# WoodsGao/pytorch_segmentation

Hardware: AMD Instinct MI355X
Metric: images/sec training step, DeepLabV3+ R50 512x512 21cl (higher is better)
Workload: dtype f32; 1 GPU; DeepLabV3+ ResNet-50 OS16, 21 classes, 512x512, batch 16 per GPU (BASELINE.json configs[2]); fwd + cross-entropy + bwd + SGD(momentum) step; global_batch=16, parallelism=dp1, conv_precision_policy=fp32, step_mode=eager

## Files before the change

### pytorch_segmentation_amd/csrc/norm_act.hip

```cpp
#include "common.h"
#include "half_io.h"

#include <stdlib.h>

namespace pseg {

constexpr int kMaxStatRows = 512;

static int stat_group(long long M, int C) {
  const int c4 = C / 4;
  const int tx = c4 >= 64 ? 64 : (c4 > 16 ? 32 : 16);
  const long long colblocks = (c4 + tx - 1) / tx;
  int r = kMaxStatRows;
  while (r > 32 && ((M + r - 1) / r) * colblocks < 1024) r >>= 1;
  return r;
}

template <typename T>
__device__ __forceinline__ f32x4 ld4(const T* p) { return ldv4(p); }
template <typename T>
__device__ __forceinline__ void st4(T* p, f32x4 v) { stv4(p, v); }

template <int V>
__device__ __forceinline__ fvec<V> act_mask_v(fvec<V> z, int act) {
// ... 74 lines not shown
}

template <int MODE, int NR, typename T, int V>
__global__ __launch_bounds__(256) void bn_bwd_reduce_kernel(const T* __restrict__ dz, int lddz,
                                                            const T* __restrict__ z, int ldz,
                                                            const T* __restrict__ y, int ldy,
                                                            const float* __restrict__ mean,
                                                            const float* __restrict__ invstd,
                                                            const float* __restrict__ scale,
                                                            const float* __restrict__ shift, int act, long long M, int C,
                                                            int R, float* __restrict__ pdb, float* __restrict__ pdg,
                                                            const uint32_t* __restrict__ mask) {
  PSEG_HELPER_PRIO();
  typedef fvec<V> vf;
  __shared__ vf sh[2][256];
  const int TX = blockDim.x, TY = blockDim.y;
  const int tx = threadIdx.x, ty = threadIdx.y;
  const int cv = blockIdx.y * TX + tx;
  const bool cok = cv * V < C;
  const long long r0 = (long long)blockIdx.x * R;
  const int nrows = (int)((r0 + R > M ? M : r0 + R) - r0);
  const int words = C >> 5;
  constexpr int ES = (int)sizeof(T);
  const __amdgpu_buffer_rsrc_t dzr = make_rsrc(dz + r0 * lddz, (uint32_t)(((long long)(nrows - 1) * lddz + C) * ES));
  const __amdgpu_buffer_rsrc_t yr = make_rsrc(y + r0 * ldy, (uint32_t)(((long long)(nrows - 1) * ldy + C) * ES));
  const __amdgpu_buffer_rsrc_t zr =
      make_rsrc(MODE == 2 ? z + r0 * ldz : y, MODE == 2 ? (uint32_t)(((long long)(nrows - 1) * ldz + C) * ES) : 0u);
  const __amdgpu_buffer_rsrc_t mr =
      make_rsrc(MODE == 1 ? mask + r0 * words : (const uint32_t*)y, MODE == 1 ? (uint32_t)(nrows * words * 4) : 0u);
  vf s = {}, q = {};
  if (cok) {
    const int c = cv * V;
    const vf mu = ldvec<V>(mean + c), is = ldvec<V>(invstd + c);
    vf sc = {}, sh4 = {};
    if (MODE == 3) {
      sc = ldvec<V>(scale + c);
      sh4 = ldvec<V>(shift + c);
    }
    const int vdz = (ty * lddz + c) * ES, vy = (ty * ldy + c) * ES, vz = (ty * ldz + c) * ES, vm = (ty * words + (c >> 5)) * 4;
    for (int base = 0; base < nrows; base += NR * TY) {
      vf g[NR], yv[NR];
#pragma unroll
      for (int k = 0; k < NR; ++k) {
        const int row = base + k * TY;
        g[k] = buf_ldvec<V, T>(dzr, vdz, row * lddz * ES);
        yv[k] = buf_ldvec<V, T>(yr, vy, row * ldy * ES);
      }
#pragma unroll
      for (int k = 0; k < NR; ++k) {
        const int row = base + k * TY;
        if (MODE == 1) {
          const uint32_t w = (uint32_t)__builtin_amdgcn_raw_buffer_load_b32(mr, vm, row * words * 4, 0);
          g[k] *= bits_to_mask<V>(w, c);
        } else if (MODE == 2) {
          g[k] *= act_mask_v<V>(buf_ldvec<V, T>(zr, vz, row * ldz * ES), act);
        } else if (MODE == 3) {
          g[k] *= act_mask_v<V>((yv[k] - mu) * sc + sh4, act);
        }
      }
      vf ts = g[0], tq = g[0] * ((yv[0] - mu) * is);
#pragma unroll
      for (int k = 1; k < NR; ++k) {
        ts += g[k];
        tq += g[k] * ((yv[k] - mu) * is);
      }
      s += ts;
      q += tq;
    }
  }
  sh[0][ty * TX + tx] = s;
  sh[1][ty * TX + tx] = q;
  __syncthreads();
  if (ty == 0 && cok) {
    vf ts = sh[0][tx], tq = sh[1][tx];
    for (int j = 1; j < TY; ++j) {
      ts += sh[0][j * TX + tx];
      tq += sh[1][j * TX + tx];
    }
    stvec<V>(pdb + (long long)blockIdx.x * C + cv * V, ts);
    stvec<V>(pdg + (long long)blockIdx.x * C + cv * V, tq);
  }
}

constexpr int kFinCh = 8, kFinLanes = 32, kFinLanesWide = 128;
constexpr int kFinWideRows = 128;

template <int LANES, int NQ>
__device__ __forceinline__ void lane_sum(double (*sh)[LANES][kFinCh], int ty, int lx, double (&v)[NQ]) {
#pragma unroll
  for (int q = 0; q < NQ; ++q) sh[q][ty][lx] = v[q];
  __syncthreads();
  constexpr int SEG = LANES >= 64 ? 16 : LANES;
  if (ty < LANES / SEG) {
#pragma unroll
    for (int q = 0; q < NQ; ++q) {
      double t = sh[q][ty * SEG][lx];
      for (int j = 1; j < SEG; ++j) t += sh[q][ty * SEG + j][lx];
      v[q] = t;
    }
  }
  if (LANES / SEG > 1) {
    __syncthreads();
    if (ty < LANES / SEG) {
#pragma unroll
      for (int q = 0; q < NQ; ++q) sh[q][ty][lx] = v[q];
    }
    __syncthreads();
    if (ty == 0) {
#pragma unroll
      for (int q = 0; q < NQ; ++q) {
        double t = sh[q][0][lx];
        for (int j = 1; j < LANES / SEG; ++j) t += sh[q][j][lx];
        v[q] = t;
      }
    }
  }
}

template <int LANES>
__device__ __forceinline__ void reduce_pair(const float* __restrict__ pa, const float* __restrict__ pb, int rows, int C,
                                            int c, int ty, double (*sh)[LANES][kFinCh], double& a, double& b) {
  const int lx = threadIdx.x % kFinCh;
  double v[2] = {0.0, 0.0};
  if (c < C) {
    int g = ty;
    for (; g + 3 * LANES < rows; g += 4 * LANES) {
      const float a0 = pa[(long long)g * C + c], a1 = pa[(long long)(g + LANES) * C + c],
                  a2 = pa[(long long)(g + 2 * LANES) * C + c], a3 = pa[(long long)(g + 3 * LANES) * C + c];
      float b0 = 0.f, b1 = 0.f, b2 = 0.f, b3 = 0.f;
      if (pb) {
        b0 = pb[(long long)g * C + c];
        b1 = pb[(long long)(g + LANES) * C + c];
        b2 = pb[(long long)(g + 2 * LANES) * C + c];
        b3 = pb[(long long)(g + 3 * LANES) * C + c];
      }
      v[0] += (double)a0;
      v[0] += (double)a1;
      v[0] += (double)a2;
      v[0] += (double)a3;
      if (pb) {
        v[1] += (double)b0;
        v[1] += (double)b1;
        v[1] += (double)b2;
        v[1] += (double)b3;
      }
    }
    for (; g < rows; g += LANES) {
      v[0] += (double)pa[(long long)g * C + c];
      if (pb) v[1] += (double)pb[(long long)g * C + c];
    }
  }
  lane_sum<LANES, 2>(sh, ty, lx, v);
  a = v[0];
  b = v[1];
}

__global__ __launch_bounds__(256) void stat_merge_kernel(const float* __restrict__ stat, int rows, int group,
                                                         long long count, int C, int per, float* __restrict__ out,
                                                         int out_rows) {
  PSEG_HELPER_PRIO();
  __shared__ double sh[2][kFinLanes][kFinCh];
  const int lx = threadIdx.x % kFinCh;
  const int c = blockIdx.x * kFinCh + lx;
  const int ty = threadIdx.x / kFinCh;
  const int g0 = blockIdx.y * per;
  int g1 = g0 + per;
  if (g1 > rows) g1 = rows;
  const long long plane = (long long)rows * C, oplane = (long long)out_rows * C;
  double s1 = 0.0, s2 = 0.0;
  float k0 = 0.f;
  if (c < C) {
    k0 = stat[(long long)g0 * C + c];
    for (int g = g0 + ty; g < g1; g += kFinLanes) {
      long long n = count - (long long)g * group;
      if (n > group) n = group;
      if (n <= 0) continue;
      const double d = (double)stat[(long long)g * C + c] - (double)k0;
      const double a = stat[plane + (long long)g * C + c], b = stat[2 * plane + (long long)g * C + c];
      s1 += a + (double)n * d;
      s2 += b + 2.0 * d * a + (double)n * d * d;
    }
  }
  sh[0][ty][lx] = s1;
  sh[1][ty][lx] = s2;
  __syncthreads();
  if (ty == 0 && c < C) {
    for (int j = 1; j < kFinLanes; ++j) {
      s1 += sh[0][j][lx];
      s2 += sh[1][j][lx];
    }
    const long long o = (long long)blockIdx.y * C + c;
    out[o] = k0;
    out[oplane + o] = (float)s1;
    out[2 * oplane + o] = (float)s2;
  }
}

template <int LANES>
__global__ __launch_bounds__(kFinCh * LANES) void bn_finalize_kernel(
    const float* __restrict__ stat, int rows, int group, long long count, int C, const float* __restrict__ gamma,
    const float* __restrict__ beta, float* __restrict__ rmean, float* __restrict__ rvar, float momentum, float eps,
    float* __restrict__ mean, float* __restrict__ invstd, float* __restrict__ scale, float* __restrict__ shift) {
  PSEG_HELPER_PRIO();
  __shared__ double sh[2][LANES][kFinCh];
  const int lx = threadIdx.x % kFinCh;
  const int c = blockIdx.x * kFinCh + lx;
  const int ty = threadIdx.x / kFinCh;
  const long long plane = (long long)rows * C;
  auto rows_of = [&](int g) -> long long {
    long long n = count - (long long)g * group;
    return n > group ? group : n;
  };
  double v[2] = {0.0, 0.0};
  double k0 = 0.0;
  if (c < C) {
    k0 = (double)stat[c];
    auto add = [&](int g, float kf, float s1f, float s2f) {
      const long long n = rows_of(g);
      if (n <= 0) return;
      const double d = (double)kf - k0, s1 = s1f;
      v[0] += s1 + (double)n * d;
      v[1] += (double)s2f + 2.0 * d * s1 + (double)n * d * d;
    };
    int g = ty;
    for (; g + 3 * LANES < rows; g += 4 * LANES) {
      float kk[4], ss1[4], ss2[4];
#pragma unroll
      for (int u = 0; u < 4; ++u) {
        const long long o = (long long)(g + u * LANES) * C + c;
        kk[u] = stat[o];
        ss1[u] = stat[plane + o];
        ss2[u] = stat[2 * plane + o];
      }
#pragma unroll
      for (int u = 0; u < 4; ++u) add(g + u * LANES, kk[u], ss1[u], ss2[u]);
    }
    for (; g < rows; g += LANES) {
      const long long o = (long long)g * C + c;
      add(g, stat[o], stat[plane + o], stat[2 * plane + o]);
    }
  }
  lane_sum<LANES, 2>(sh, ty, lx, v);
  if (ty == 0 && c < C) {
    const double n = (double)count;
    const double mu = k0 + v[0] / n;
    double M2 = v[1] - v[0] * v[0] / n;
    if (M2 < 0.0) M2 = 0.0;
    const double var = M2 / n;
    const float is = (float)(1.0 / sqrt(var + (double)eps));
    const float g = gamma ? gamma[c] : 1.f, b = beta ? beta[c] : 0.f;
    const float fm = (float)mu;
    mean[c] = fm;
    invstd[c] = is;
    const float sc = g * is;
    scale[c] = sc;
    shift[c] = b;
    if (rmean) rmean[c] = (1.f - momentum) * rmean[c] + momentum * fm;
    if (rvar) {
      const double unbiased = count > 1 ? M2 / (n - 1.0) : var;
      rvar[c] = (1.f - momentum) * rvar[c] + momentum * (float)unbiased;
    }
  }
}

template <int LANES>
__global__ __launch_bounds__(kFinCh * LANES) void bn_bwd_finalize_kernel(
    const float* __restrict__ pdb, const float* __restrict__ pdg, int rows, long long count, int C,
    float* __restrict__ dgamma, float* __restrict__ dbeta, int accumulate, int frozen, float* __restrict__ c1,
    float* __restrict__ c2) {
  PSEG_HELPER_PRIO();
  __shared__ double sh[2][LANES][kFinCh];
  const int c = blockIdx.x * kFinCh + (threadIdx.x % kFinCh);
  const int ty = threadIdx.x / kFinCh;
  double db, dg;
  reduce_pair<LANES>(pdb, pdg, rows, C, c, ty, sh, db, dg);
  if (ty == 0 && c < C) {
    const float fdb = (float)db, fdg = (float)dg;
    if (dbeta) dbeta[c] = accumulate ? dbeta[c] + fdb : fdb;
    if (dgamma) dgamma[c] = accumulate ? dgamma[c] + fdg : fdg;
    c1[c] = frozen ? 0.f : (float)(db / (double)count);
    c2[c] = frozen ? 0.f : (float)(dg / (double)count);
  }
}

template <int LANES>
__global__ __launch_bounds__(kFinCh * LANES) void col_reduce_kernel(const float* __restrict__ part, int rows, int C,
                                                                    float* __restrict__ out, int accumulate) {
  PSEG_HELPER_PRIO();
  __shared__ double sh[2][LANES][kFinCh];
  const int c = blockIdx.x * kFinCh + (threadIdx.x % kFinCh);
  const int ty = threadIdx.x / kFinCh;
  double s, unused;
  reduce_pair<LANES>(part, nullptr, rows, C, c, ty, sh, s, unused);
  if (ty == 0 && c < C) out[c] = accumulate ? out[c] + (float)s : (float)s;
}

__global__ void bn_eval_coeffs_kernel(const float* __restrict__ gamma, const float* __restrict__ beta,
                                      const float* __restrict__ rmean, const float* __restrict__ rvar, float eps, int C,
                                      float* __restrict__ mean, float* __restrict__ invstd, float* __restrict__ scale,
                                      float* __restrict__ shift) {
  PSEG_HELPER_PRIO();
  const int c = blockIdx.x * blockDim.x + threadIdx.x;
  if (c < C) {
    const float is = 1.f / sqrtf(rvar[c] + eps);
    mean[c] = rmean[c];
    invstd[c] = is;
    scale[c] = (gamma ? gamma[c] : 1.f) * is;
    shift[c] = beta ? beta[c] : 0.f;
  }
}

template <typename T, int V>
__global__ __launch_bounds__(256) void bn_act_fwd_kernel(const T* __restrict__ y, int ldy,
                                                         const float* __restrict__ mean, const float* __restrict__ scale,
                                                         const float* __restrict__ shift,
                                                         const T* __restrict__ res, int ldr, int act,
                                                         T* __restrict__ z, int ldz, uint32_t total, FastDiv cvdiv,
                                                         unsigned* __restrict__ amax, uint32_t* __restrict__ maskout) {
  PSEG_HELPER_PRIO();
  typedef fvec<V> vf;
  float vmax = 0.f;
  for (uint32_t i = blockIdx.x * 256u + threadIdx.x; i < total; i += gridDim.x * 256u) {
    const uint32_t r = cvdiv.div(i);
    const uint32_t c = (i - r * cvdiv.d) * V;
    vf v = ldvec<V>(y + (long long)r * ldy + c);
    if (scale) v = (v - ldvec<V>(mean + c)) * ldvec<V>(scale + c) + ldvec<V>(shift + c);
    if (res) v += ldvec<V>(res + (long long)r * ldr + c);
    if (maskout != nullptr) {
      vf vs = v;
      if constexpr (sizeof(T) == 2) vs = __builtin_convertvector(__builtin_convertvector(v, f16x8v), vf);
      const vf m = act_mask_v<V>(vs, act);
      uint32_t bits = 0;
#pragma unroll
      for (int k = 0; k < V; ++k) bits |= (m[k] != 0.f ? 1u : 0u) << k;
      bits <<= (c & 31);
#pragma unroll
      for (int o = 1; o < 32 / V; o <<= 1) bits |= __shfl_xor(bits, o, 64);
      if ((threadIdx.x & (32 / V - 1)) == 0) maskout[(long long)r * ((cvdiv.d * V) >> 5) + (c >> 5)] = bits;
    }
    if (act == PSEG_ACT_RELU) {
#pragma unroll
      for (int k = 0; k < V; ++k) v[k] = fmaxf(v[k], 0.f);
    } else if (act == PSEG_ACT_RELU6) {
#pragma unroll
      for (int k = 0; k < V; ++k) v[k] = fminf(fmaxf(v[k], 0.f), 6.f);
    }
    stvec<V>(z + (long long)r * ldz + c, v);
#pragma unroll
    for (int k = 0; k < V; ++k) vmax = fmaxf(vmax, fabsf(v[k]));
  }
  if (amax != nullptr) {
    __shared__ float shm[4];
#pragma unroll
    for (int o = 32; o > 0; o >>= 1) vmax = fmaxf(vmax, __shfl_xor(vmax, o, 64));
    if ((threadIdx.x & 63) == 0) shm[threadIdx.x >> 6] = vmax;
    __syncthreads();
    if (threadIdx.x == 0) {
      const float m = fmaxf(fmaxf(shm[0], shm[1]), fmaxf(shm[2], shm[3]));
      publish_amax(amax, m);
    }
  }
}

template <int NR, typename T, int V>
__global__ __launch_bounds__(256) void bn_act_fwd_rows_kernel(const T* __restrict__ y, int ldy,
                                                              const float* __restrict__ mean, const float* __restrict__ scale,
                                                              const float* __restrict__ shift, const T* __restrict__ res,
                                                              int ldr, int act, T* __restrict__ z, int ldz, long long M, int C,
                                                              int RB, uint32_t* __restrict__ maskout) {
  PSEG_HELPER_PRIO();
  typedef fvec<V> vf;
  const int TX = blockDim.x, TY = blockDim.y;
  const int tx = threadIdx.x, ty = threadIdx.y;
  const int cv = blockIdx.y * TX + tx;
  if (cv * V >= C) return;
  const int c = cv * V;
  const long long r0 = (long long)blockIdx.x * RB;
// ... 282 lines not shown
  {
    const int ch = threadIdx.x & (kSmallCh - 1), q = threadIdx.x / kSmallCh;
    const int c = c0 + ch;
    const bool cok = c < C;
    if (cok)
      for (int j = q; j < kFinLanes; j += 256 / kSmallCh) {
        double a = 0.0, b = 0.0;
        for (int g = j; g < rows; g += kFinLanes) {
          a += (double)pdb[(long long)g * C + c];
          b += (double)pdg[(long long)g * C + c];
        }
        s_pa[ch][j] = a;
        s_pb[ch][j] = b;
      }
    __syncthreads();
    if (q == 0) {
      float c1 = 0.f, c2 = 0.f;
      if (cok) {
        double db = 0.0, dg = 0.0;
        for (int j = 0; j < kFinLanes; ++j) {
          db += s_pa[ch][j];
          dg += s_pb[ch][j];
        }
        const float fdb = (float)db, fdg = (float)dg;
        if (blockIdx.x == 0) {
          if (dbeta) dbeta[c] = accumulate ? dbeta[c] + fdb : fdb;
          if (dgamma) dgamma[c] = accumulate ? dgamma[c] + fdg : fdg;
        }
        c1 = frozen ? 0.f : (float)(db / (double)count);
        c2 = frozen ? 0.f : (float)(dg / (double)count);
      }
      s_c1[ch] = c1;
      s_c2[ch] = c2;
    }
  }
  __syncthreads();
  const int tx = threadIdx.x & 15, ty = threadIdx.x >> 4;
  const int c = c0 + tx * 4;
  if (c >= C) return;
  const f32x4 c1 = ld4(&s_c1[tx * 4]), c2 = ld4(&s_c2[tx * 4]);
  const f32x4 mu = ld4(mean + c), is = ld4(invstd + c), sc = ld4(scale + c);
  f32x4 sh = {0.f, 0.f, 0.f, 0.f};
  if (shift) sh = ld4(shift + c);
  const long long r0 = (long long)blockIdx.x * kSmallRowsPerBlock;
  long long r1 = r0 + kSmallRowsPerBlock;
  if (r1 > M) r1 = M;
  for (long long r = r0 + ty; r < r1; r += 16) {
    f32x4 g = ld4(dz + r * lddz + c);
    const f32x4 yv = ld4(y + r * ldy + c);
    if (act != PSEG_ACT_NONE) g *= act_mask(z != nullptr ? ld4(z + r * ldz + c) : (yv - mu) * sc + sh, act);
    if (dres) {
      T* dp = dres + r * lddres + c;
      st4(dp, res_acc ? ld4(dp) + g : g);
    }
    const f32x4 xh = (yv - mu) * is;
    st4(dy + r * lddy + c, sc * (g - c1 - xh * c2));
  }
}

static bool al16(const void* p) { return ((uintptr_t)p & 15) == 0; }

static void stat_block(int C, dim3& block, dim3& grid, long long M, int R, int V = 4) {
  const int cv = C / V;
  const int tx = cv >= 64 ? 64 : (cv > 16 ? 32 : (cv > 8 ? 16 : 8));
  block = dim3(tx, 256 / tx);
  grid = dim3((unsigned)cdiv(M, R), (unsigned)cdiv(cv, tx));
}

template <typename T>
constexpr int lane_channels() { return sizeof(T) == 2 ? 8 : 4; }

static int ew_grid(long long total) {
  long long b = (total + 255) / 256;
  if (b > 256 * 8) b = 256 * 8;
  if (b < 1) b = 1;
  return (int)b;
}

#define EW_COMMON_CHECKS(name, M, C)                                                              \
  PSEG_REQUIRE((M) > 0 && (C) > 0 && (C) % 4 == 0, name ": need M > 0, C %% 4 == 0 (M=%lld C=%d)", \
               (long long)(M), (int)(C));                                                         \
  PSEG_REQUIRE((long long)(M) * ((C) / 4) < (1LL << 31), name ": tensor too large")

int launch_col_reduce(const float* part, int rows, int C, float* out, int accumulate, hipStream_t st) {
  if (rows >= kFinWideRows)
    hipLaunchKernelGGL(col_reduce_kernel<kFinLanesWide>, dim3(cdiv(C, kFinCh)), dim3(kFinCh * kFinLanesWide), 0, st, part,
                       rows, C, out, accumulate);
  else
    hipLaunchKernelGGL(col_reduce_kernel<kFinLanes>, dim3(cdiv(C, kFinCh)), dim3(kFinCh * kFinLanes), 0, st, part, rows, C,
                       out, accumulate);
  PSEG_LAUNCH_CHECK();
  return PSEG_OK;
}


template <typename T>
static bool ld_ok(int ld) { return ld % (sizeof(T) == 2 ? 8 : 4) == 0; }

template <typename T>
static int col_stats_impl(const T* y, int ldy, int64_t M, int C, float* stat, void* stream) {
  PSEG_REQUIRE(y && stat, "col_stats: null pointer");
  EW_COMMON_CHECKS("col_stats", M, C);
  PSEG_REQUIRE(ld_ok<T>(ldy) && al16(y) && al16(stat), "col_stats: alignment");
  dim3 block, grid;
  const int R = stat_group(M, C);
  stat_block(C, block, grid, M, R);
  hipLaunchKernelGGL((col_stats_kernel<true, T>), grid, block, 0, (hipStream_t)stream, y, ldy, (long long)M, C, R, stat,
                     (long long)cdiv(M, R) * C);
  PSEG_LAUNCH_CHECK();
  return PSEG_OK;
}

template <typename T>
static int bn_fwd_fused_impl(const float* stat, int rows, int group, int64_t count, int C, const float* gamma,
                             const float* beta, float* running_mean, float* running_var, float momentum, float eps,
                             float* mean, float* invstd, float* scale, float* shift, const T* y, int ldy, const T* residual,
                             int ldr, int act, T* z, int ldz, int64_t M, float* amax_z, void* stream) {
  PSEG_REQUIRE(stat && mean && invstd && scale && shift && y && z, "bn_fwd_fused: null pointer");
  PSEG_REQUIRE(rows > 0 && rows <= kSmallMaxPartials && group > 0 && count > 0, "bn_fwd_fused: bad sizes (rows %d)", rows);
  PSEG_REQUIRE((long long)rows * group >= count, "bn_fwd_fused: groups do not cover the rows");
  EW_COMMON_CHECKS("bn_fwd_fused", M, C);
  PSEG_REQUIRE(ld_ok<T>(ldy) && ld_ok<T>(ldz) && (!residual || ld_ok<T>(ldr)) && al16(y) && al16(z) && al16(residual),
               "bn_fwd_fused: alignment");
  const dim3 grid((unsigned)cdiv(M, kSmallRowsPerBlock), (unsigned)cdiv(C, kSmallCh));
  hipLaunchKernelGGL(bn_fwd_small_kernel<T>, grid, dim3(256), 0, (hipStream_t)stream, stat, rows, group, (long long)count,
                     C, gamma, beta, running_mean, running_var, momentum, eps, mean, invstd, scale, shift, y, ldy, residual,
                     ldr, act, z, ldz, (long long)M, (unsigned*)amax_z);
  PSEG_LAUNCH_CHECK();
  return PSEG_OK;
}

template <typename T>
static int bn_bwd_fused_impl(const float* part_db, const float* part_dg, int rows, int64_t count, int C, float* dgamma,
                             float* dbeta, int accumulate, int frozen, const T* dz, int lddz, const T* z, int ldz,
                             const T* y, int ldy, const float* mean, const float* invstd, const float* scale,
                             const float* shift, int act, T* dy, int lddy, T* dres, int lddres, int res_accumulate,
                             int64_t M, void* stream) {
  PSEG_REQUIRE(part_db && part_dg && dz && y && mean && invstd && scale && dy, "bn_bwd_fused: null pointer");
  PSEG_REQUIRE(rows > 0 && count > 0, "bn_bwd_fused: bad sizes");
  PSEG_REQUIRE(act == PSEG_ACT_NONE || z || shift, "bn_bwd_fused: activation needs z or shift");
  EW_COMMON_CHECKS("bn_bwd_fused", M, C);
  PSEG_REQUIRE(ld_ok<T>(lddz) && ld_ok<T>(ldy) && ld_ok<T>(lddy) && (!z || ld_ok<T>(ldz)) && (!dres || ld_ok<T>(lddres)) &&
                   al16(dz) && al16(z) && al16(y) && al16(dy) && al16(dres),
               "bn_bwd_fused: alignment");
  const dim3 grid((unsigned)cdiv(M, kSmallRowsPerBlock), (unsigned)cdiv(C, kSmallCh));
  hipLaunchKernelGGL(bn_bwd_small_kernel<T>, grid, dim3(256), 0, (hipStream_t)stream, part_db, part_dg, rows,
                     (long long)count, C, dgamma, dbeta, accumulate, frozen, dz, lddz, z, ldz, y, ldy, mean, invstd, scale,
                     shift, act, dy, lddy, dres, lddres, res_accumulate, (long long)M);
  PSEG_LAUNCH_CHECK();
  return PSEG_OK;
}

template <typename T>
static int bn_act_fwd_impl(const T* y, int ldy, const float* mean, const float* scale, const float* shift, const T* residual,
                           int ldr, int act, T* z, int ldz, int64_t M, int C, float* amax_z, uint32_t* mask_out,
                           void* stream) {
  PSEG_REQUIRE(y && z, "bn_act_fwd: null pointer");
  PSEG_REQUIRE(mask_out == nullptr || (C % 32 == 0 && act != PSEG_ACT_NONE), "bn_act_fwd: mask_out needs C %% 32 == 0 and an activation");
  PSEG_REQUIRE((scale == nullptr) == (shift == nullptr) && (scale == nullptr) == (mean == nullptr),
               "bn_act_fwd: mean/scale/shift must come together");
  EW_COMMON_CHECKS("bn_act_fwd", M, C);
  PSEG_REQUIRE(ld_ok<T>(ldy) && ld_ok<T>(ldz) && (!residual || ld_ok<T>(ldr)) && al16(y) && al16(z) && al16(residual) &&
                   al16(mean) && al16(scale) && al16(shift),
               "bn_act_fwd: alignment");
  constexpr int V = lane_channels<T>();
  const uint32_t total = (uint32_t)(M * (C / V));
  static const int rows_mode = [] {
    const char* e = getenv("PSEG_BN_FWD_ROWS");
    return e ? atoi(e) : 1;
  }();
  if constexpr (sizeof(T) == 2) {
    if (rows_mode != 0 && scale != nullptr && amax_z == nullptr && C % 8 == 0 && M >= 256 && (residual == nullptr || rows_mode == 2)) {
      dim3 block, grid;
// ... 95 lines not shown
                   al16(z) && al16(dy) && al16(dres) && al16(scale),
               "act_bwd: alignment");
  const uint32_t total = (uint32_t)(M * (C / 4));
  hipLaunchKernelGGL(act_bwd_kernel<T>, dim3(ew_grid(total)), dim3(256), 0, (hipStream_t)stream, dz, lddz, z, ldz, scale, act,
                     dy, lddy, dres, lddres, res_accumulate, total, FastDiv((uint32_t)(C / 4)));
  PSEG_LAUNCH_CHECK();
  return PSEG_OK;
}

template <typename T>
static int col_sum_impl(const T* dy, int ldy, int64_t M, int C, float* out, int accumulate, void* workspace,
                        int64_t workspace_bytes, void* stream) {
  PSEG_REQUIRE(dy && out, "col_sum: null pointer");
  EW_COMMON_CHECKS("col_sum", M, C);
  PSEG_REQUIRE(ld_ok<T>(ldy) && al16(dy) && al16(workspace), "col_sum: alignment");
  const int R = stat_group(M, C);
  const int rows = cdiv(M, R);
  const long long need = (long long)rows * C * 4;
  if (!workspace || workspace_bytes < need) {
    set_error("col_sum: needs %lld workspace bytes, got %lld", need, (long long)workspace_bytes);
    return PSEG_ERR_WORKSPACE;
  }
  dim3 block, grid;
  stat_block(C, block, grid, M, R);
  hipLaunchKernelGGL((col_stats_kernel<false, T>), grid, block, 0, (hipStream_t)stream, dy, ldy, (long long)M, C, R,
                     (float*)workspace, 0LL);
  PSEG_LAUNCH_CHECK();
  return launch_col_reduce((const float*)workspace, rows, C, out, accumulate, (hipStream_t)stream);
}

template <typename T>
static int copy2d_impl(const T* x, int ldx, T* y, int ldy, int64_t M, int C, int accumulate, void* stream) {
  PSEG_REQUIRE(x && y, "copy2d: null pointer");
  EW_COMMON_CHECKS("copy2d", M, C);
  PSEG_REQUIRE(ld_ok<T>(ldx) && ld_ok<T>(ldy) && al16(x) && al16(y), "copy2d: alignment");
  const uint32_t total = (uint32_t)(M * (C / 4));
  hipLaunchKernelGGL(copy2d_kernel<T>, dim3(ew_grid(total)), dim3(256), 0, (hipStream_t)stream, x, ldx, y, ldy, accumulate,
                     total, FastDiv((uint32_t)(C / 4)));
  PSEG_LAUNCH_CHECK();
  return PSEG_OK;
}

}

using namespace pseg;

#define HP(p) reinterpret_cast<const half_t*>(p)
#define HPM(p) reinterpret_cast<half_t*>(p)

extern "C" {

int pseg_col_stats_rows(int64_t M, int C) { return cdiv(M, stat_group(M, C)); }

int pseg_col_stats_group(int64_t M, int C) { return stat_group(M, C); }

int pseg_col_stats(const float* y, int ldy, int64_t M, int C, float* stat, void* stream) {
  return col_stats_impl<float>(y, ldy, M, C, stat, stream);
}
int pseg_col_stats_h(const pseg_half_t* y, int ldy, int64_t M, int C, float* stat, void* stream) {
  return col_stats_impl<half_t>(HP(y), ldy, M, C, stat, stream);
}

constexpr int kMergePer = 64;
constexpr int kTwoStageRows = 2048;

int64_t pseg_bn_finalize_workspace_bytes(int rows, int C) {
  return rows > kTwoStageRows ? (int64_t)3 * cdiv(rows, kMergePer) * C * 4 : 0;
}

int pseg_bn_finalize(const float* stat, int rows, int group, int64_t count, int C, const float* gamma,
                     const float* beta, float* running_mean, float* running_var, float momentum, float eps, float* mean,
                     float* invstd, float* scale, float* shift, void* workspace, int64_t workspace_bytes, void* stream) {
  PSEG_REQUIRE(stat && mean && invstd && scale && shift, "bn_finalize: null pointer");
  PSEG_REQUIRE(rows > 0 && group > 0 && count > 0 && C > 0, "bn_finalize: bad sizes");
  PSEG_REQUIRE((long long)rows * group >= count, "bn_finalize: %d groups of %d rows do not cover %lld rows", rows, group,
               (long long)count);
  if (rows > kTwoStageRows) {
    const int64_t need = pseg_bn_finalize_workspace_bytes(rows, C);
    if (!workspace || workspace_bytes < need) {
      set_error("bn_finalize: needs %lld workspace bytes, got %lld", (long long)need, (long long)workspace_bytes);
      return PSEG_ERR_WORKSPACE;
    }
    const int out_rows = cdiv(rows, kMergePer);
    hipLaunchKernelGGL(stat_merge_kernel, dim3(cdiv(C, kFinCh), out_rows), dim3(256), 0, (hipStream_t)stream, stat, rows,
                       group, (long long)count, C, kMergePer, (float*)workspace, out_rows);
    PSEG_LAUNCH_CHECK();
    stat = (const float*)workspace;
    rows = out_rows;
    group *= kMergePer;
  }
  if (rows >= kFinWideRows)
    hipLaunchKernelGGL(bn_finalize_kernel<kFinLanesWide>, dim3(cdiv(C, kFinCh)), dim3(kFinCh * kFinLanesWide), 0,
                       (hipStream_t)stream, stat, rows, group, (long long)count, C, gamma, beta, running_mean, running_var,
                       momentum, eps, mean, invstd, scale, shift);
  else
    hipLaunchKernelGGL(bn_finalize_kernel<kFinLanes>, dim3(cdiv(C, kFinCh)), dim3(kFinCh * kFinLanes), 0,
                       (hipStream_t)stream, stat, rows, group, (long long)count, C, gamma, beta, running_mean, running_var,
                       momentum, eps, mean, invstd, scale, shift);
  PSEG_LAUNCH_CHECK();
  return PSEG_OK;
}

int pseg_bn_small_path(int rows, int64_t M, int C) {
  static const int mode = [] {
    const char* e = getenv("PSEG_BN_SMALL");
    return e ? atoi(e) : 1;
  }();
  if (mode == 0) return 0;
  return (rows > 0 && rows <= kSmallMaxPartials && M * (int64_t)C <= (int64_t)(8 << 20)) ? 1 : 0;
}

int pseg_bn_fwd_fused(const float* stat, int rows, int group, int64_t count, int C, const float* gamma, const float* beta,
                      float* running_mean, float* running_var, float momentum, float eps, float* mean, float* invstd,
                      float* scale, float* shift, const float* y, int ldy, const float* residual, int ldr, int act,
                      float* z, int ldz, int64_t M, float* amax_z, void* stream) {
  return bn_fwd_fused_impl<float>(stat, rows, group, count, C, gamma, beta, running_mean, running_var, momentum, eps, mean,
                                  invstd, scale, shift, y, ldy, residual, ldr, act, z, ldz, M, amax_z, stream);
}
int pseg_bn_fwd_fused_h(const float* stat, int rows, int group, int64_t count, int C, const float* gamma, const float* beta,
                        float* running_mean, float* running_var, float momentum, float eps, float* mean, float* invstd,
                        float* scale, float* shift, const pseg_half_t* y, int ldy, const pseg_half_t* residual, int ldr,
                        int act, pseg_half_t* z, int ldz, int64_t M, void* stream) {
  return bn_fwd_fused_impl<half_t>(stat, rows, group, count, C, gamma, beta, running_mean, running_var, momentum, eps, mean,
                                   invstd, scale, shift, HP(y), ldy, HP(residual), ldr, act, HPM(z), ldz, M, nullptr, stream);
}

int pseg_bn_bwd_fused(const float* part_db, const float* part_dg, int rows, int64_t count, int C, float* dgamma,
                      float* dbeta, int accumulate, int frozen, const float* dz, int lddz, const float* z, int ldz,
                      const float* y, int ldy, const float* mean, const float* invstd, const float* scale,
                      const float* shift, int act, float* dy, int lddy, float* dres, int lddres, int res_accumulate,
                      int64_t M, void* stream) {
  return bn_bwd_fused_impl<float>(part_db, part_dg, rows, count, C, dgamma, dbeta, accumulate, frozen, dz, lddz, z, ldz, y,
                                  ldy, mean, invstd, scale, shift, act, dy, lddy, dres, lddres, res_accumulate, M, stream);
}
int pseg_bn_bwd_fused_h(const float* part_db, const float* part_dg, int rows, int64_t count, int C, float* dgamma,
                        float* dbeta, int accumulate, int frozen, const pseg_half_t* dz, int lddz, const pseg_half_t* z,
                        int ldz, const pseg_half_t* y, int ldy, const float* mean, const float* invstd, const float* scale,
                        const float* shift, int act, pseg_half_t* dy, int lddy, pseg_half_t* dres, int lddres,
                        int res_accumulate, int64_t M, void* stream) {
  return bn_bwd_fused_impl<half_t>(part_db, part_dg, rows, count, C, dgamma, dbeta, accumulate, frozen, HP(dz), lddz, HP(z),
                                   ldz, HP(y), ldy, mean, invstd, scale, shift, act, HPM(dy), lddy, HPM(dres), lddres,
                                   res_accumulate, M, stream);
}

int pseg_bn_eval_coeffs(const float* gamma, const float* beta, const float* running_mean, const float* running_var,
                        float eps, int C, float* mean, float* invstd, float* scale, float* shift, void* stream) {
  PSEG_REQUIRE(running_mean && running_var && mean && invstd && scale && shift && C > 0, "bn_eval_coeffs: bad argument");
  hipLaunchKernelGGL(bn_eval_coeffs_kernel, dim3(cdiv(C, 256)), dim3(256), 0, (hipStream_t)stream, gamma, beta,
                     running_mean, running_var, eps, C, mean, invstd, scale, shift);
  PSEG_LAUNCH_CHECK();
  return PSEG_OK;
}

int pseg_bn_act_fwd(const float* y, int ldy, const float* mean, const float* scale, const float* shift,
                    const float* residual, int ldr, int act, float* z, int ldz, int64_t M, int C, float* amax_z,
                    uint32_t* mask_out, void* stream) {
  return bn_act_fwd_impl<float>(y, ldy, mean, scale, shift, residual, ldr, act, z, ldz, M, C, amax_z, mask_out, stream);
}
int pseg_bn_act_fwd_h(const pseg_half_t* y, int ldy, const float* mean, const float* scale, const float* shift,
                      const pseg_half_t* residual, int ldr, int act, pseg_half_t* z, int ldz, int64_t M, int C,
                      uint32_t* mask_out, void* stream) {
  return bn_act_fwd_impl<half_t>(HP(y), ldy, mean, scale, shift, HP(residual), ldr, act, HPM(z), ldz, M, C, nullptr,
                                 mask_out, stream);
}

int pseg_bn_act_bwd_reduce(const float* dz, int lddz, const float* z, int ldz, const float* y, int ldy, const float* mean,
                           const float* invstd, const float* scale, const float* shift, int act, int64_t M, int C,
                           float* part_db, float* part_dg, const uint32_t* mask, void* stream) {
  return bn_act_bwd_reduce_impl<float>(dz, lddz, z, ldz, y, ldy, mean, invstd, scale, shift, act, M, C, part_db, part_dg,
                                       mask, stream);
}
int pseg_bn_act_bwd_reduce_h(const pseg_half_t* dz, int lddz, const pseg_half_t* z, int ldz, const pseg_half_t* y, int ldy,
                             const float* mean, const float* invstd, const float* scale, const float* shift, int act,
                             int64_t M, int C, float* part_db, float* part_dg, const uint32_t* mask, void* stream) {
  return bn_act_bwd_reduce_impl<half_t>(HP(dz), lddz, HP(z), ldz, HP(y), ldy, mean, invstd, scale, shift, act, M, C, part_db,
                                        part_dg, mask, stream);
}

int pseg_bn_bwd_finalize(const float* part_db, const float* part_dg, int rows, int64_t count, int C, float* dgamma,
                         float* dbeta, int accumulate, int frozen, float* c1, float* c2, void* stream) {
  PSEG_REQUIRE(part_db && part_dg && c1 && c2 && rows > 0 && count > 0 && C > 0, "bn_bwd_finalize: bad argument");
  if (rows >= kFinWideRows)
    hipLaunchKernelGGL(bn_bwd_finalize_kernel<kFinLanesWide>, dim3(cdiv(C, kFinCh)), dim3(kFinCh * kFinLanesWide), 0,
                       (hipStream_t)stream, part_db, part_dg, rows, (long long)count, C, dgamma, dbeta, accumulate, frozen, c1,
                       c2);
  else
    hipLaunchKernelGGL(bn_bwd_finalize_kernel<kFinLanes>, dim3(cdiv(C, kFinCh)), dim3(kFinCh * kFinLanes), 0,
                       (hipStream_t)stream, part_db, part_dg, rows, (long long)count, C, dgamma, dbeta, accumulate, frozen, c1,
                       c2);
  PSEG_LAUNCH_CHECK();
  return PSEG_OK;
}

int pseg_bn_act_bwd_apply(const float* dz, int lddz, const float* z, int ldz, const float* y, int ldy, const float* mean,
                          const float* invstd, const float* scale, const float* shift, const float* c1, const float* c2,
                          int act, float* dy, int lddy, float* dres, int lddres, int res_accumulate, int64_t M, int C,
                          const uint32_t* mask, uint16_t* dy_hi, uint16_t* dy_lo, int ldp, void* stream) {
  return bn_act_bwd_apply_impl<float>(dz, lddz, z, ldz, y, ldy, mean, invstd, scale, shift, c1, c2, act, dy, lddy, dres,
                                      lddres, res_accumulate, M, C, mask, dy_hi, dy_lo, ldp, stream);
}
int pseg_bn_act_bwd_apply_h(const pseg_half_t* dz, int lddz, const pseg_half_t* z, int ldz, const pseg_half_t* y, int ldy,
                            const float* mean, const float* invstd, const float* scale, const float* shift, const float* c1,
                            const float* c2, int act, pseg_half_t* dy, int lddy, pseg_half_t* dres, int lddres,
                            int res_accumulate, int64_t M, int C, const uint32_t* mask, void* stream) {
  return bn_act_bwd_apply_impl<half_t>(HP(dz), lddz, HP(z), ldz, HP(y), ldy, mean, invstd, scale, shift, c1, c2, act, HPM(dy),
                                       lddy, HPM(dres), lddres, res_accumulate, M, C, mask, nullptr, nullptr, 0, stream);
}

int pseg_act_bwd(const float* dz, int lddz, const float* z, int ldz, const float* scale, int act, float* dy, int lddy,
                 float* dres, int lddres, int res_accumulate, int64_t M, int C, void* stream) {
  return act_bwd_impl<float>(dz, lddz, z, ldz, scale, act, dy, lddy, dres, lddres, res_accumulate, M, C, stream);
}
int pseg_act_bwd_h(const pseg_half_t* dz, int lddz, const pseg_half_t* z, int ldz, const float* scale, int act,
                   pseg_half_t* dy, int lddy, pseg_half_t* dres, int lddres, int res_accumulate, int64_t M, int C,
                   void* stream) {
  return act_bwd_impl<half_t>(HP(dz), lddz, HP(z), ldz, scale, act, HPM(dy), lddy, HPM(dres), lddres, res_accumulate, M, C,
                              stream);
}

int pseg_col_sum(const float* dy, int ldy, int64_t M, int C, float* out, int accumulate, void* workspace,
                 int64_t workspace_bytes, void* stream) {
  return col_sum_impl<float>(dy, ldy, M, C, out, accumulate, workspace, workspace_bytes, stream);
}
int pseg_col_sum_h(const pseg_half_t* dy, int ldy, int64_t M, int C, float* out, int accumulate, void* workspace,
                   int64_t workspace_bytes, void* stream) {
  return col_sum_impl<half_t>(HP(dy), ldy, M, C, out, accumulate, workspace, workspace_bytes, stream);
}

int pseg_copy2d(const float* x, int ldx, float* y, int ldy, int64_t M, int C, int accumulate, void* stream) {
  return copy2d_impl<float>(x, ldx, y, ldy, M, C, accumulate, stream);
}
int pseg_copy2d_h(const pseg_half_t* x, int ldx, pseg_half_t* y, int ldy, int64_t M, int C, int accumulate, void* stream) {
  return copy2d_impl<half_t>(HP(x), ldx, HPM(y), ldy, M, C, accumulate, stream);
}

}
```

Baseline: 372.2 images/sec.

## Restructure BN finalize reductions with row-major lanes, float4 loads and wave shuffles

Reworks the batch-norm statistic merge, finalize, backward-finalize and column-reduce kernels so each lane walks rows for a group of channels. Loads become 16-byte vectors where C is divisible by 4 and pointers are aligned. Row counts are bucketed into compile-time unrolled variants so all loads issue before the double-precision accumulation. Cross-lane sums use wave shuffles instead of multi-stage shared-memory loops. The aim is to cut latency of these small launch-bound helper kernels that run for every BN layer, at the cost of many more template instantiations and more complex clamped-index and masking logic.

```diff
diff --git a/pytorch_segmentation_amd/csrc/norm_act.hip b/pytorch_segmentation_amd/csrc/norm_act.hip
--- a/pytorch_segmentation_amd/csrc/norm_act.hip
+++ b/pytorch_segmentation_amd/csrc/norm_act.hip
@@ -180,217 +180,303 @@
   }
 }
 
-constexpr int kFinCh = 8, kFinLanes = 32, kFinLanesWide = 128;
+constexpr int kFinThreads = 256, kFinLanes = 32, kFinLanesWide = 128;
 constexpr int kFinWideRows = 128;
 
-template <int LANES, int NQ>
-__device__ __forceinline__ void lane_sum(double (*sh)[LANES][kFinCh], int ty, int lx, double (&v)[NQ]) {
-#pragma unroll
-  for (int q = 0; q < NQ; ++q) sh[q][ty][lx] = v[q];
-  __syncthreads();
-  constexpr int SEG = LANES >= 64 ? 16 : LANES;
-  if (ty < LANES / SEG) {
-#pragma unroll
-    for (int q = 0; q < NQ; ++q) {
-      double t = sh[q][ty * SEG][lx];
-      for (int j = 1; j < SEG; ++j) t += sh[q][ty * SEG + j][lx];
-      v[q] = t;
-    }
-  }
-  if (LANES / SEG > 1) {
+template <int V>
+struct FinVec {
+  float x[V];
+};
+template <int V>
+__device__ __forceinline__ FinVec<V> fin_ld(const float* __restrict__ p) {
+  FinVec<V> r;
+  if constexpr (V == 4) {
+    const f32x4 t = *reinterpret_cast<const f32x4*>(p);
+    r.x[0] = t[0];
+    r.x[1] = t[1];
+    r.x[2] = t[2];
+    r.x[3] = t[3];
+  } else {
+    static_assert(V == 1, "one or four channels per lane");
+    r.x[0] = *p;
+  }
+  return r;
+}
+
+template <int LANES, int V>
+struct FinShape {
+  static constexpr int CG = kFinThreads / LANES;
+  static constexpr int CH = CG * V;
+  static constexpr int STRIDE = LANES + 1;
+  template <int NQ>
+  static constexpr int lds() { return LANES == kFinLanesWide ? (kFinThreads / 64) * NQ * V : NQ * V * CG * STRIDE; }
+};
+
+template <int LANES, int V, int NQ>
+__device__ __forceinline__ void lane_sum(double (&v)[NQ][V], double* __restrict__ sh, double (&out)[NQ]) {
+  typedef FinShape<LANES, V> S;
+  const int tid = threadIdx.x;
+  if constexpr (LANES == kFinLanesWide) {
+#pragma unroll
+    for (int o = 32; o > 0; o >>= 1) {
+#pragma unroll
+      for (int q = 0; q < NQ; ++q)
+#pragma unroll
+        for (int k = 0; k < V; ++k) v[q][k] += __shfl_xor(v[q][k], o, 64);
+    }
+    if ((tid & 63) == 0) {
+#pragma unroll
+      for (int q = 0; q < NQ; ++q)
+#pragma unroll
+        for (int k = 0; k < V; ++k) sh[(tid >> 6) * (NQ * V) + q * V + k] = v[q][k];
+    }
     __syncthreads();
-    if (ty < LANES / SEG) {
-#pragma unroll
-      for (int q = 0; q < NQ; ++q) sh[q][ty][lx] = v[q];
-    }
+    if (tid < S::CH) {
+      const int w = (tid / V) * (LANES / 64), k = tid % V;
+#pragma unroll
+      for (int q = 0; q < NQ; ++q) out[q] = sh[w * (NQ * V) + q * V + k] + sh[(w + 1) * (NQ * V) + q * V + k];
+    }
+  } else {
+    static_assert(NQ * S::CH <= 64, "one wave adds the lane sums");
+    const int ty = tid % LANES, cg = tid / LANES;
+#pragma unroll
+    for (int q = 0; q < NQ; ++q)
+#pragma unroll
+      for (int k = 0; k < V; ++k) sh[((q * V + k) * S::CG + cg) * S::STRIDE + ty] = v[q][k];
     __syncthreads();
-    if (ty == 0) {
-#pragma unroll
-      for (int q = 0; q < NQ; ++q) {
-        double t = sh[q][0][lx];
-        for (int j = 1; j < LANES / SEG; ++j) t += sh[q][j][lx];
-        v[q] = t;
-      }
-    }
-  }
-}
-
-template <int LANES>
-__device__ __forceinline__ void reduce_pair(const float* __restrict__ pa, const float* __restrict__ pb, int rows, int C,
-                                            int c, int ty, double (*sh)[LANES][kFinCh], double& a, double& b) {
-  const int lx = threadIdx.x % kFinCh;
-  double v[2] = {0.0, 0.0};
-  if (c < C) {
-    int g = ty;
-    for (; g + 3 * LANES < rows; g += 4 * LANES) {
-      const float a0 = pa[(long long)g * C + c], a1 = pa[(long long)(g + LANES) * C + c],
-                  a2 = pa[(long long)(g + 2 * LANES) * C + c], a3 = pa[(long long)(g + 3 * LANES) * C + c];
-      float b0 = 0.f, b1 = 0.f, b2 = 0.f, b3 = 0.f;
-      if (pb) {
-        b0 = pb[(long long)g * C + c];
-        b1 = pb[(long long)(g + LANES) * C + c];
-        b2 = pb[(long long)(g + 2 * LANES) * C + c];
-        b3 = pb[(long long)(g + 3 * LANES) * C + c];
-      }
-      v[0] += (double)a0;
-      v[0] += (double)a1;
-      v[0] += (double)a2;
-      v[0] += (double)a3;
-      if (pb) {
-        v[1] += (double)b0;
-        v[1] += (double)b1;
-        v[1] += (double)b2;
-        v[1] += (double)b3;
-      }
-    }
-    for (; g < rows; g += LANES) {
-      v[0] += (double)pa[(long long)g * C + c];
-      if (pb) v[1] += (double)pb[(long long)g * C + c];
-    }
-  }
-  lane_sum<LANES, 2>(sh, ty, lx, v);
-  a = v[0];
-  b = v[1];
-}
-
-__global__ __launch_bounds__(256) void stat_merge_kernel(const float* __restrict__ stat, int rows, int group,
-                                                         long long count, int C, int per, float* __restrict__ out,
-                                                         int out_rows) {
+    if (tid < 64) {
+      double t = 0.0;
+      if (tid < NQ * S::CH) {
+        const int ch = tid % S::CH, q = tid / S::CH;
+        const double* p = sh + ((q * V + ch % V) * S::CG + ch / V) * S::STRIDE;
+        t = p[0];
+#pragma unroll 8
+        for (int j = 1; j < LANES; ++j) t += p[j];
+      }
+#pragma unroll
+      for (int q = 0; q < NQ; ++q) out[q] = __shfl(t, (tid % S::CH) + q * S::CH, 64);
+    }
+  }
+}
+
+static int fin_bucket(int rows, int lanes) {
+  for (int nr = 2; nr <= 16; nr *= 2)
+    if (rows <= nr * lanes) return nr;
+  return 0;
+}
+
+template <int LANES, int V, int NR, int NQ>
+__device__ __forceinline__ void reduce_rows(const float* __restrict__ pa, const float* __restrict__ pb, int rows, int C,
+                                            int cv, int ty, double (&v)[NQ][V]) {
+  constexpr int B = NR > 0 ? NR : 4;
+  for (int base = 0; base < (NR > 0 ? 1 : rows); base += B * LANES) {
+    FinVec<V> a[B], b[NQ == 2 ? B : 1];
+#pragma unroll
+    for (int u = 0; u < B; ++u) {
+      const int g = base + ty + u * LANES;
+      const long long o = (long long)(g < rows ? g : rows - 1) * C + cv;
+      a[u] = fin_ld<V>(pa + o);
+      if constexpr (NQ == 2) b[u] = fin_ld<V>(pb + o);
+    }
+    __builtin_amdgcn_sched_barrier(0);
+#pragma unroll
+    for (int u = 0; u < B; ++u) {
+      const bool ok = base + ty + u * LANES < rows;
+#pragma unroll
+      for (int k = 0; k < V; ++k) {
+        v[0][k] += (double)(ok ? a[u].x[k] : 0.f);
+        if constexpr (NQ == 2) v[1][k] += (double)(ok ? b[u].x[k] : 0.f);
+      }
+    }
+  }
+}
+
+template <int V>
+__global__ __launch_bounds__(kFinThreads) void stat_merge_kernel(const float* __restrict__ stat, int rows, int group,
+                                                                 long long count, int C, float* __restrict__ out,
+                                                                 int out_rows) {
   PSEG_HELPER_PRIO();
-  __shared__ double sh[2][kFinLanes][kFinCh];
-  const int lx = threadIdx.x % kFinCh;
-  const int c = blockIdx.x * kFinCh + lx;
-  const int ty = threadIdx.x / kFinCh;
+  constexpr int NR = 2, per = NR * kFinLanes;
+  const int ty = threadIdx.x % kFinLanes;
+  const int cv = (blockIdx.x * (kFinThreads / kFinLanes) + threadIdx.x / kFinLanes) * V;
   const int g0 = blockIdx.y * per;
-  int g1 = g0 + per;
-  if (g1 > rows) g1 = rows;
+  const int g1 = g0 + per < rows ? g0 + per : rows;
   const long long plane = (long long)rows * C, oplane = (long long)out_rows * C;
-  double s1 = 0.0, s2 = 0.0;
-  float k0 = 0.f;
-  if (c < C) {
-    k0 = stat[(long long)g0 * C + c];
-    for (int g = g0 + ty; g < g1; g += kFinLanes) {
+  double s1[V], s2[V];
+#pragma unroll
+  for (int k = 0; k < V; ++k) s1[k] = s2[k] = 0.0;
+  FinVec<V> k0 = {};
+  if (cv < C) {
+    FinVec<V> kk[NR], a[NR], b[NR];
+    k0 = fin_ld<V>(stat + (long long)g0 * C + cv);
+#pragma unroll
+    for (int u = 0; u < NR; ++u) {
+      const int g = g0 + ty + u * kFinLanes;
+      const long long o = (long long)(g < g1 ? g : g1 - 1) * C + cv;
+      kk[u] = fin_ld<V>(stat + o);
+      a[u] = fin_ld<V>(stat + plane + o);
+      b[u] = fin_ld<V>(stat + 2 * plane + o);
+    }
+    __builtin_amdgcn_sched_barrier(0);
+#pragma unroll
+    for (int u = 0; u < NR; ++u) {
+      const int g = g0 + ty + u * kFinLanes;
       long long n = count - (long long)g * group;
       if (n > group) n = group;
-      if (n <= 0) continue;
-      const double d = (double)stat[(long long)g * C + c] - (double)k0;
-      const double a = stat[plane + (long long)g * C + c], b = stat[2 * plane + (long long)g * C + c];
-      s1 += a + (double)n * d;
-      s2 += b + 2.0 * d * a + (double)n * d * d;
-    }
-  }
-  sh[0][ty][lx] = s1;
-  sh[1][ty][lx] = s2;
-  __syncthreads();
-  if (ty == 0 && c < C) {
-    for (int j = 1; j < kFinLanes; ++j) {
-      s1 += sh[0][j][lx];
-      s2 += sh[1][j][lx];
-    }
-    const long long o = (long long)blockIdx.y * C + c;
-    out[o] = k0;
-    out[oplane + o] = (float)s1;
-    out[2 * oplane + o] = (float)s2;
-  }
-}
-
-template <int LANES>
-__global__ __launch_bounds__(kFinCh * LANES) void bn_finalize_kernel(
+      const bool ok = g < g1 && n > 0;
+      if (!ok) n = 0;
+#pragma unroll
+      for (int k = 0; k < V; ++k) {
+        const double d = (double)(ok ? kk[u].x[k] : k0.x[k]) - (double)k0.x[k], sa = ok ? a[u].x[k] : 0.f;
+        s1[k] += sa + (double)n * d;
+        s2[k] += (double)(ok ? b[u].x[k] : 0.f) + 2.0 * d * sa + (double)n * d * d;
+      }
+    }
+  }
+#pragma unroll
+  for (int o = kFinLanes / 2; o > 0; o >>= 1) {
+#pragma unroll
+    for (int k = 0; k < V; ++k) {
+      s1[k] += __shfl_xor(s1[k], o, 64);
+      s2[k] += __shfl_xor(s2[k], o, 64);
+    }
+  }
+  if (ty == 0 && cv < C) {
+    const long long o = (long long)blockIdx.y * C + cv;
+#pragma unroll
+    for (int k = 0; k < V; ++k) {
+      out[o + k] = k0.x[k];
+      out[oplane + o + k] = (float)s1[k];
+      out[2 * oplane + o + k] = (float)s2[k];
+    }
+  }
+}
+
+template <int LANES, int V, int NR>
+__global__ __launch_bounds__(kFinThreads) void bn_finalize_kernel(
     const float* __restrict__ stat, int rows, int group, long long count, int C, const float* __restrict__ gamma,
     const float* __restrict__ beta, float* __restrict__ rmean, float* __restrict__ rvar, float momentum, float eps,
     float* __restrict__ mean, float* __restrict__ invstd, float* __restrict__ scale, float* __restrict__ shift) {
   PSEG_HELPER_PRIO();
-  __shared__ double sh[2][LANES][kFinCh];
-  const int lx = threadIdx.x % kFinCh;
-  const int c = blockIdx.x * kFinCh + lx;
-  const int ty = threadIdx.x / kFinCh;
+  typedef FinShape<LANES, V> S;
+  __shared__ double sh[S::template lds<2>()];
+  const int ty = threadIdx.x % LANES;
+  const int cv = blockIdx.x * S::CH + (threadIdx.x / LANES) * V;
+  const int c = blockIdx.x * S::CH + threadIdx.x;
+  const bool fin = threadIdx.x < S::CH && c < C;
   const long long plane = (long long)rows * C;
-  auto rows_of = [&](int g) -> long long {
-    long long n = count - (long long)g * group;
-    return n > group ? group : n;
-  };
-  double v[2] = {0.0, 0.0};
-  double k0 = 0.0;
-  if (c < C) {
-    k0 = (double)stat[c];
-    auto add = [&](int g, float kf, float s1f, float s2f) {
-      const long long n = rows_of(g);
-      if (n <= 0) return;
-      const double d = (double)kf - k0, s1 = s1f;
-      v[0] += s1 + (double)n * d;
-      v[1] += (double)s2f + 2.0 * d * s1 + (double)n * d * d;
-    };
-    int g = ty;
-    for (; g + 3 * LANES < rows; g += 4 * LANES) {
-      float kk[4], ss1[4], ss2[4];
-#pragma unroll
-      for (int u = 0; u < 4; ++u) {
-        const long long o = (long long)(g + u * LANES) * C + c;
-        kk[u] = stat[o];
-        ss1[u] = stat[plane + o];
-        ss2[u] = stat[2 * plane + o];
-      }
-#pragma unroll
-      for (int u = 0; u < 4; ++u) add(g + u * LANES, kk[u], ss1[u], ss2[u]);
-    }
-    for (; g < rows; g += LANES) {
-      const long long o = (long long)g * C + c;
-      add(g, stat[o], stat[plane + o], stat[2 * plane + o]);
-    }
-  }
-  lane_sum<LANES, 2>(sh, ty, lx, v);
-  if (ty == 0 && c < C) {
+  float ek0 = 0.f, eg = 1.f, eb = 0.f, erm = 0.f, erv = 0.f;
+  if (fin) {
+    ek0 = stat[c];
+    if (gamma) eg = gamma[c];
+    if (beta) eb = beta[c];
+    if (rmean) erm = rmean[c];
+    if (rvar) erv = rvar[c];
+  }
+  double v[2][V];
+#pragma unroll
+  for (int k = 0; k < V; ++k) v[0][k] = v[1][k] = 0.0;
+  if (cv < C) {
+    constexpr int B = NR > 0 ? NR : 4;
+    const FinVec<V> k0 = fin_ld<V>(stat + cv);
+    for (int base = 0; base < (NR > 0 ? 1 : rows); base += B * LANES) {
+      FinVec<V> kk[B], a[B], b[B];
+#pragma unroll
+      for (int u = 0; u < B; ++u) {
+        const int g = base + ty + u * LANES;
+        const long long o = (long long)(g < rows ? g : rows - 1) * C + cv;
+        kk[u] = fin_ld<V>(stat + o);
+        a[u] = fin_ld<V>(stat + plane + o);
+        b[u] = fin_ld<V>(stat + 2 * plane + o);
+      }
+      __builtin_amdgcn_sched_barrier(0);
+#pragma unroll
+      for (int u = 0; u < B; ++u) {
+        const int g = base + ty + u * LANES;
+        long long n = count - (long long)g * group;
+        if (n > group) n = group;
+        const bool ok = g < rows && n > 0;
+        if (!ok) n = 0;
+#pragma unroll
+        for (int k = 0; k < V; ++k) {
+          const double d = (double)(ok ? kk[u].x[k] : k0.x[k]) - (double)k0.x[k], s1 = ok ? a[u].x[k] : 0.f;
+          v[0][k] += s1 + (double)n * d;
+          v[1][k] += (double)(ok ? b[u].x[k] : 0.f) + 2.0 * d * s1 + (double)n * d * d;
+        }
+      }
+    }
+  }
+  double s[2];
+  lane_sum<LANES, V, 2>(v, sh, s);
+  if (fin) {
     const double n = (double)count;
-    const double mu = k0 + v[0] / n;
-    double M2 = v[1] - v[0] * v[0] / n;
+    const double mu = (double)ek0 + s[0] / n;
+    double M2 = s[1] - s[0] * s[0] / n;
     if (M2 < 0.0) M2 = 0.0;
     const double var = M2 / n;
     const float is = (float)(1.0 / sqrt(var + (double)eps));
-    const float g = gamma ? gamma[c] : 1.f, b = beta ? beta[c] : 0.f;
     const float fm = (float)mu;
     mean[c] = fm;
     invstd[c] = is;
-    const float sc = g * is;
-    scale[c] = sc;
-    shift[c] = b;
-    if (rmean) rmean[c] = (1.f - momentum) * rmean[c] + momentum * fm;
+    scale[c] = eg * is;
+    shift[c] = eb;
+    if (rmean) rmean[c] = (1.f - momentum) * erm + momentum * fm;
     if (rvar) {
       const double unbiased = count > 1 ? M2 / (n - 1.0) : var;
-      rvar[c] = (1.f - momentum) * rvar[c] + momentum * (float)unbiased;
-    }
-  }
-}
-
-template <int LANES>
-__global__ __launch_bounds__(kFinCh * LANES) void bn_bwd_finalize_kernel(
+      rvar[c] = (1.f - momentum) * erv + momentum * (float)unbiased;
+    }
+  }
+}
+
+template <int LANES, int V, int NR>
+__global__ __launch_bounds__(kFinThreads) void bn_bwd_finalize_kernel(
     const float* __restrict__ pdb, const float* __restrict__ pdg, int rows, long long count, int C,
     float* __restrict__ dgamma, float* __restrict__ dbeta, int accumulate, int frozen, float* __restrict__ c1,
     float* __restrict__ c2) {
   PSEG_HELPER_PRIO();
-  __shared__ double sh[2][LANES][kFinCh];
-  const int c = blockIdx.x * kFinCh + (threadIdx.x % kFinCh);
-  const int ty = threadIdx.x / kFinCh;
-  double db, dg;
-  reduce_pair<LANES>(pdb, pdg, rows, C, c, ty, sh, db, dg);
-  if (ty == 0 && c < C) {
-    const float fdb = (float)db, fdg = (float)dg;
-    if (dbeta) dbeta[c] = accumulate ? dbeta[c] + fdb : fdb;
-    if (dgamma) dgamma[c] = accumulate ? dgamma[c] + fdg : fdg;
-    c1[c] = frozen ? 0.f : (float)(db / (double)count);
-    c2[c] = frozen ? 0.f : (float)(dg / (double)count);
-  }
-}
-
-template <int LANES>
-__global__ __launch_bounds__(kFinCh * LANES) void col_reduce_kernel(const float* __restrict__ part, int rows, int C,
-                                                                    float* __restrict__ out, int accumulate) {
+  typedef FinShape<LANES, V> S;
+  __shared__ double sh[S::template lds<2>()];
+  const int cv = blockIdx.x * S::CH + (threadIdx.x / LANES) * V;
+  const int c = blockIdx.x * S::CH + threadIdx.x;
+  const bool fin = threadIdx.x < S::CH && c < C;
+  float eb = 0.f, eg = 0.f;
+  if (fin && accumulate) {
+    if (dbeta) eb = dbeta[c];
+    if (dgamma) eg = dgamma[c];
+  }
+  double v[2][V];
+#pragma unroll
+  for (int k = 0; k < V; ++k) v[0][k] = v[1][k] = 0.0;
+  if (cv < C) reduce_rows<LANES, V, NR, 2>(pdb, pdg, rows, C, cv, threadIdx.x % LANES, v);
+  double s[2];
+  lane_sum<LANES, V, 2>(v, sh, s);
+  if (fin) {
+    const float fdb = (float)s[0], fdg = (float)s[1];
+    if (dbeta) dbeta[c] = accumulate ? eb + fdb : fdb;
+    if (dgamma) dgamma[c] = accumulate ? eg + fdg : fdg;
+    c1[c] = frozen ? 0.f : (float)(s[0] / (double)count);
+    c2[c] = frozen ? 0.f : (float)(s[1] / (double)count);
+  }
+}
+
+template <int LANES, int V, int NR>
+__global__ __launch_bounds__(kFinThreads) void col_reduce_kernel(const float* __restrict__ part, int rows, int C,
+                                                                 float* __restrict__ out, int accumulate) {
   PSEG_HELPER_PRIO();
-  __shared__ double sh[2][LANES][kFinCh];
-  const int c = blockIdx.x * kFinCh + (threadIdx.x % kFinCh);
-  const int ty = threadIdx.x / kFinCh;
-  double s, unused;
-  reduce_pair<LANES>(part, nullptr, rows, C, c, ty, sh, s, unused);
-  if (ty == 0 && c < C) out[c] = accumulate ? out[c] + (float)s : (float)s;
+  typedef FinShape<LANES, V> S;
+  __shared__ double sh[S::template lds<1>()];
+  const int cv = blockIdx.x * S::CH + (threadIdx.x / LANES) * V;
+  const int c = blockIdx.x * S::CH + threadIdx.x;
+  const bool fin = threadIdx.x < S::CH && c < C;
+  float e = 0.f;
+  if (fin && accumulate) e = out[c];
+  double v[1][V];
+#pragma unroll
+  for (int k = 0; k < V; ++k) v[0][k] = 0.0;
+  if (cv < C) reduce_rows<LANES, V, NR, 1>(part, nullptr, rows, C, cv, threadIdx.x % LANES, v);
+  double s[1];
+  lane_sum<LANES, V, 1>(v, sh, s);
+  if (fin) out[c] = accumulate ? e + (float)s[0] : (float)s[0];
 }
 
 __global__ void bn_eval_coeffs_kernel(const float* __restrict__ gamma, const float* __restrict__ beta,
@@ -839,13 +925,40 @@
                (long long)(M), (int)(C));                                                         \
   PSEG_REQUIRE((long long)(M) * ((C) / 4) < (1LL << 31), name ": tensor too large")
 
+static bool fin_vec_ok(int C, const void* a, const void* b = nullptr) { return C % 4 == 0 && al16(a) && al16(b); }
+
+template <int L, int V, int NR>
+struct FinSel {
+  static constexpr int lanes = L, vec = V, nr = NR;
+  static constexpr int ch = FinShape<L, V>::CH;
+};
+template <typename F>
+static void fin_dispatch(int rows, bool vec, F&& f) {
+  const bool wide = rows >= kFinWideRows;
+  const int nr = vec ? fin_bucket(rows, wide ? kFinLanesWide : kFinLanes) : 0;
+  if (!vec) {
+    if (wide) f(FinSel<kFinLanesWide, 1, 0>());
+    else f(FinSel<kFinLanes, 1, 0>());
+  } else if (wide) {
+    switch (nr) {
+      case 2: f(FinSel<kFinLanesWide, 4, 2>()); break;
+      case 4: f(FinSel<kFinLanesWide, 4, 4>()); break;
+      case 8: f(FinSel<kFinLanesWide, 4, 8>()); break;
+      case 16: f(FinSel<kFinLanesWide, 4, 16>()); break;
+      default: f(FinSel<kFinLanesWide, 4, 0>()); break;
+    }
+  } else {
+    if (nr == 2) f(FinSel<kFinLanes, 4, 2>());
+    else f(FinSel<kFinLanes, 4, 4>());
+  }
+}
+
 int launch_col_reduce(const float* part, int rows, int C, float* out, int accumulate, hipStream_t st) {
-  if (rows >= kFinWideRows)
-    hipLaunchKernelGGL(col_reduce_kernel<kFinLanesWide>, dim3(cdiv(C, kFinCh)), dim3(kFinCh * kFinLanesWide), 0, st, part,
+  fin_dispatch(rows, fin_vec_ok(C, part), [&](auto s) {
+    typedef decltype(s) S;
+    hipLaunchKernelGGL((col_reduce_kernel<S::lanes, S::vec, S::nr>), dim3(cdiv(C, S::ch)), dim3(kFinThreads), 0, st, part,
                        rows, C, out, accumulate);
-  else
-    hipLaunchKernelGGL(col_reduce_kernel<kFinLanes>, dim3(cdiv(C, kFinCh)), dim3(kFinCh * kFinLanes), 0, st, part, rows, C,
-                       out, accumulate);
+  });
   PSEG_LAUNCH_CHECK();
   return PSEG_OK;
 }
@@ -1107,21 +1220,25 @@
       return PSEG_ERR_WORKSPACE;
     }
     const int out_rows = cdiv(rows, kMergePer);
-    hipLaunchKernelGGL(stat_merge_kernel, dim3(cdiv(C, kFinCh), out_rows), dim3(256), 0, (hipStream_t)stream, stat, rows,
-                       group, (long long)count, C, kMergePer, (float*)workspace, out_rows);
+    static_assert(kMergePer == 2 * kFinLanes, "stat_merge_kernel: two groups per lane");
+    constexpr int cg = kFinThreads / kFinLanes;
+    if (fin_vec_ok(C, stat, workspace))
+      hipLaunchKernelGGL(stat_merge_kernel<4>, dim3(cdiv(C, 4 * cg), out_rows), dim3(kFinThreads), 0, (hipStream_t)stream,
+                         stat, rows, group, (long long)count, C, (float*)workspace, out_rows);
+    else
+      hipLaunchKernelGGL(stat_merge_kernel<1>, dim3(cdiv(C, cg), out_rows), dim3(kFinThreads), 0, (hipStream_t)stream, stat,
+                         rows, group, (long long)count, C, (float*)workspace, out_rows);
     PSEG_LAUNCH_CHECK();
     stat = (const float*)workspace;
     rows = out_rows;
     group *= kMergePer;
   }
-  if (rows >= kFinWideRows)
-    hipLaunchKernelGGL(bn_finalize_kernel<kFinLanesWide>, dim3(cdiv(C, kFinCh)), dim3(kFinCh * kFinLanesWide), 0,
+  fin_dispatch(rows, fin_vec_ok(C, stat), [&](auto s) {
+    typedef decltype(s) S;
+    hipLaunchKernelGGL((bn_finalize_kernel<S::lanes, S::vec, S::nr>), dim3(cdiv(C, S::ch)), dim3(kFinThreads), 0,
                        (hipStream_t)stream, stat, rows, group, (long long)count, C, gamma, beta, running_mean, running_var,
                        momentum, eps, mean, invstd, scale, shift);
-  else
-    hipLaunchKernelGGL(bn_finalize_kernel<kFinLanes>, dim3(cdiv(C, kFinCh)), dim3(kFinCh * kFinLanes), 0,
-                       (hipStream_t)stream, stat, rows, group, (long long)count, C, gamma, beta, running_mean, running_var,
-                       momentum, eps, mean, invstd, scale, shift);
+  });
   PSEG_LAUNCH_CHECK();
   return PSEG_OK;
 }
@@ -1205,14 +1322,12 @@
 int pseg_bn_bwd_finalize(const float* part_db, const float* part_dg, int rows, int64_t count, int C, float* dgamma,
                          float* dbeta, int accumulate, int frozen, float* c1, float* c2, void* stream) {
   PSEG_REQUIRE(part_db && part_dg && c1 && c2 && rows > 0 && count > 0 && C > 0, "bn_bwd_finalize: bad argument");
-  if (rows >= kFinWideRows)
-    hipLaunchKernelGGL(bn_bwd_finalize_kernel<kFinLanesWide>, dim3(cdiv(C, kFinCh)), dim3(kFinCh * kFinLanesWide), 0,
+  fin_dispatch(rows, fin_vec_ok(C, part_db, part_dg), [&](auto s) {
+    typedef decltype(s) S;
+    hipLaunchKernelGGL((bn_bwd_finalize_kernel<S::lanes, S::vec, S::nr>), dim3(cdiv(C, S::ch)), dim3(kFinThreads), 0,
                        (hipStream_t)stream, part_db, part_dg, rows, (long long)count, C, dgamma, dbeta, accumulate, frozen, c1,
                        c2);
-  else
-    hipLaunchKernelGGL(bn_bwd_finalize_kernel<kFinLanes>, dim3(cdiv(C, kFinCh)), dim3(kFinCh * kFinLanes), 0,
-                       (hipStream_t)stream, part_db, part_dg, rows, (long long)count, C, dgamma, dbeta, accumulate, frozen, c1,
-                       c2);
+  });
   PSEG_LAUNCH_CHECK();
   return PSEG_OK;
 }
```

Result: no change. 371.6 images/sec (-0.1%).
